# zhouxuguang/GNXRayTracer

Measured on AMD Instinct MI355X. Metric: Mrays/sec + wall-clock to 1024spp, dragon Cornell 1920×1080, higher is better.
Workload: dtype f32; 1 GPU; cfg3: Cornell + synthetic 100000-tri mesh (stand-in for absent dragon.3d), Glass+Metal, PathIntegrator maxDepth 8 rr 1 spatial, Halton(1024), 1920x1080; passes_in_flight=4, sub_passes=56, spp_rendered=1024, gather=n/a, world_size=1, backend=none, devices_visible=1

## Files before the change

### gnxraytracer_amd/csrc/api_render.hip.h

```cpp
#pragma once

struct TraceLaunch {
    int entries;
    int lds_entries;
    bool spill_needed;
    size_t lds;
    int n_top;
    int blocks;
};
static TraceLaunch trace_launch(const gnxr_scene *s, bool wide, bool spheres, long long total) {
    TraceLaunch t;
    t.entries = wide ? s->cs.stack4_need + 1 : s->cs.bvh_max_depth + 2;
    const int per_cu = g_trace_blocks_per_cu;
    const size_t fixed_b = wide ? (size_t)(kRayRecDwords + (spheres ? 1 : 0)) * kRqStride * sizeof(int) + (size_t)kTopCache * 128 + 128 : 0;
    t.lds_entries = std::min(std::min(t.entries, Knobs::trace_lds_levels()), std::max(2, (int)(((160 * 1024) / per_cu - 1024 - fixed_b) / (kBlock * sizeof(int)))));
    t.spill_needed = t.entries > t.lds_entries;
    t.lds = (size_t)t.lds_entries * kBlock * sizeof(int) + fixed_b;
    t.n_top = (int)std::min<size_t>(kTopCache, s->cs.root4 >= 0 ? s->cs.nodes4.size() : 0);
    t.blocks = (int)std::min<long long>((long long)g_num_cus * per_cu, (total + kBlock - 1) / kBlock);
    return t;
}

static int count_local_rows(const gnxr_render_params *p) {
    int rows = 0;
// ... 144 lines not shown
        return GNXR_ERR_INVALID;
    }
    return GNXR_OK;
}

int RenderState::reserve(const RenderPlan &pl) {
    const size_t cap = pl.cap, nrec = pl.nrec;
    int rc;
#define AL(f) if ((rc = f.alloc(cap)) != GNXR_OK) return rc;
    for (int i = 0; i < kRecGroups; ++i) {
        const size_t per_slot = i < 2 ? 1 : (i < 4 ? nrec : (pl.direct ? nrec : 1));
        if ((rc = rec[i].alloc(cap * per_slot * kRS)) != GNXR_OK) return rc;
    }
    if ((rc = mis_Y.alloc(cap * (pl.direct ? nrec : 1))) != GNXR_OK) return rc;
    AL(L) AL(hit) AL(queue_a) AL(queue_b) AL(queue_nee) AL(queue_c0) AL(queue_c1) AL(queue_c2) AL(queue_c3) AL(pflags) AL(pclass) AL(nee_vis)
    if (pl.whitted) {
        const size_t nl = (size_t)std::max(1, pl.n_records), md = (size_t)std::max(1, pl.p.max_depth);
        if ((rc = wh_rec.alloc(cap * nl)) ||
            (rc = wh_o.alloc(cap * md)) || (rc = wh_d.alloc(cap * md)) || (rc = wh_L.alloc(cap * md)) || (rc = wh_w.alloc(cap * md)) ||
            (rc = wh_pdf.alloc(cap * md)) || (rc = vol_vs.alloc(cap)))
            return rc;
        if (pl.textured_scene && ((rc = wh_rxo.alloc(cap * (md + 1))) || (rc = wh_rxd.alloc(cap * (md + 1))) || (rc = wh_ryo.alloc(cap * (md + 1))) || (rc = wh_ryd.alloc(cap * (md + 1)))))
            return rc;
    }
    if (pl.volpath) {
        AL(vol_n1) AL(vol_f) AL(vol_Li) AL(vol_Tr) AL(vol_Ld) AL(vol_mres) AL(vol_vs) AL(vol_state)
        AL(vol_Lout) AL(vol_alt_state) AL(vol_orig) AL(vol_alt_orig) AL(vol_newslot)
        for (int i = 0; i < kVolPackF4; ++i) AL(vol_alt[i])
        for (int i = 0; i < kRecGroups; ++i) if ((rc = vol_alt_rec[i].alloc(cap * kRS)) != GNXR_OK) return rc;
    }
#undef AL
    if ((rc = trace_spill.alloc((size_t)g_num_cus * g_trace_blocks_per_cu * kBlock * (size_t)pl.spill_entries * 2)) != GNXR_OK) return rc;
    if (!pl.caller_rays && (rc = accum.alloc(pl.npix)) != GNXR_OK) return rc;
    const int max_tiles = (int)((cap + kCompactTile - 1) / kCompactTile);
    if ((rc = tile_counts.alloc((size_t)5 * max_tiles)) != GNXR_OK) return rc;
    if (pl.n_views > 0 && (rc = view_cams.alloc((size_t)pl.n_views)) != GNXR_OK) return rc;
    return GNXR_OK;
}

unsigned long long RenderState::state_bytes(const RenderPlan &pl) {
    const unsigned long long per_slot = (2ull * kRecGroups + 2) * sizeof(float4) + 8ull * sizeof(int) + 2 + sizeof(unsigned int);
    return (unsigned long long)pl.cap * per_slot + (pl.volpath ? (unsigned long long)pl.cap * (6ull * sizeof(float4) + sizeof(int4) + 1) : 0ull);
}

PathArrays RenderState::path_arrays() {
    PathArrays pa;
    float4 *rec_primary[kRecGroups];
    record_ptrs(rec, rec_primary);
    pa.bind_records(rec_primary);
    pa.mis_Y = mis_Y.p;
    pa.L = L.p; pa.hit = hit.p; pa.pflags = pflags.p; pa.pclass = pclass.p; pa.nee_vis = nee_vis.p;
    return pa;
}
VolArrays RenderState::vol_arrays() {
    VolArrays va;
    float4 *rec_primary[kRecGroups];
    record_ptrs(rec, rec_primary);
    va.bind_records(rec_primary);
    va.mis_Y = mis_Y.p;
    va.vs = vol_vs.p; va.n1 = vol_n1.p; va.f = vol_f.p;
    va.Li = vol_Li.p; va.Tr = vol_Tr.p; va.Ld = vol_Ld.p; va.mres = vol_mres.p; va.state = vol_state.p;
    va.orig = vol_orig.p; va.Lout = vol_Lout.p;
    return va;
}
WhittedArrays RenderState::whitted_arrays(const RenderPlan &pl, int n_lights) {
    WhittedArrays wa;
    wa.ws = vol_vs.p; wa.fr_o = wh_o.p; wa.fr_d = wh_d.p; wa.fr_L = wh_L.p; wa.fr_w = wh_w.p; wa.fr_pdf = wh_pdf.p;
    wa.fr_rxo = wh_rxo.p; wa.fr_rxd = wh_rxd.p; wa.fr_ryo = wh_ryo.p; wa.fr_ryd = wh_ryd.p;
    wa.cap = (int)pl.cap; wa.n_lights = n_lights; wa.n_records = pl.n_records;
    wa.start_dim = pl.wmode == WM_DIRECT_ALL ? 5 + 2 * (pl.p.max_depth * n_lights * 2) : 5;
    return wa;
}
VolPackSet RenderState::pack_set(bool alt) {
    VolPackSet ps;
    if (!alt) {
// ... 68 lines not shown
        const int dlds_entries = std::min(std::min(entries, Knobs::trace_lds_levels()), std::max(2, (int)(((160 * 1024) / dper_cu - 1024 - dfixed) / (2 * kBlock * sizeof(int)))));
        const int dspill_levels = std::max(0, entries - dlds_entries);
        const size_t dlds = (size_t)2 * dlds_entries * kBlock * sizeof(int) + dfixed;
        const int dn_top = (int)std::min<size_t>(kTopCacheD, s->cs.root4 >= 0 ? s->cs.nodes4.size() : 0);
        const int dblocks = (int)std::min<long long>((long long)g_num_cus * dper_cu, (total + 2 * kBlock - 1) / (2 * kBlock));
#define GX_TRACE4D(S, P) hipLaunchKernelGGL((k_trace4d<S, P>), dim3(std::max(1, dblocks)), dim3(kBlock), dlds, stream, sc, pa, w, &dctr->cursor, dctr, dlds_entries, dspill_levels, st.trace_spill.p, chunk, dn_top)
        if (spheres) { if (dspill_levels > 0) GX_TRACE4D(true, true); else GX_TRACE4D(true, false); }
        else { if (dspill_levels > 0) GX_TRACE4D(false, true); else GX_TRACE4D(false, false); }
#undef GX_TRACE4D
    } else
#endif
    if (wide) {
        if (spheres) { if (count_wide) GX_TRACE4_CS(true, true); else GX_TRACE4_CS(false, true); }
        else { if (count_wide) GX_TRACE4_CS(true, false); else GX_TRACE4_CS(false, false); }
    } else {
        const bool cnt = counting || count_wide;
        if (spheres) { if (cnt) GX_TRACE(true, false, true); else GX_TRACE(false, false, true); }
        else { if (cnt) GX_TRACE(true, false, false); else GX_TRACE(false, false, false); }
    }
#undef GX_TRACE4_CS
#undef GX_TRACE4
#undef GX_TRACE
    if (timing) timer.end(stream);
    if (count_rays) {
        rays_closest += (unsigned long long)w.n_closest + (unsigned long long)n_mis;
        rays_any += (unsigned long long)n_sh;
        rays_mis += (unsigned long long)n_mis;
    }
    ++launches;
}

void RenderRun::compact(int mode, const int *qin, int nin, const unsigned char *keys, int nout, int nscatter, unsigned int *totals, int *o0, int *o1, int *o2, int *o3, int split,
                        const unsigned *n_dev) {
    int tiles = (nin + kCompactTile - 1) / kCompactTile;
    int g = std::max(1, std::min(tiles, g_num_cus * g_grid_bpc));
    unsigned int *tc = st.tile_counts.p;
    const bool hitclass = mode == COMPACT_HITCLASS;
    const int *hit = hitclass ? (const int *)st.hit.p : nullptr;
    const unsigned char *cls = hitclass ? (const unsigned char *)s->tri_class.p : nullptr;
    unsigned char *keys_out = hitclass ? st.pclass.p : nullptr;
#define GX_COUNT(M, N, SPLIT) hipLaunchKernelGGL((k_compact_count<M, N>), dim3(g), dim3(kCompactBlock), 0, stream, qin, nin, keys, tc, tiles, hit, cls, keys_out, SPLIT, n_dev)
#define GX_SCATTER(M, N, O3) hipLaunchKernelGGL((k_compact_scatter<M, N>), dim3(g), dim3(kCompactBlock), 0, stream, qin, nin, keys, (const unsigned int *)tc, tiles, o0, o1, o2, O3, n_dev)
    if (mode == COMPACT_FLAGS && nout == 5) GX_COUNT(COMPACT_FLAGS, 5, split);
    else if (mode == COMPACT_FLAGS) GX_COUNT(COMPACT_FLAGS, 4, 0);
    else if (hitclass) { if (nout == 4) GX_COUNT(COMPACT_HITCLASS, 4, 0); else GX_COUNT(COMPACT_HITCLASS, 3, 0); }
    else if (nout == 4) GX_COUNT(COMPACT_CLASS, 4, 0);
    else GX_COUNT(COMPACT_CLASS, 3, 0);
    hipLaunchKernelGGL(k_compact_scan, dim3(nout), dim3(1024), 0, stream, tc, tiles, totals, n_dev);
    if (mode == COMPACT_FLAGS && nscatter == 3) GX_SCATTER(COMPACT_FLAGS, 3, (int *)nullptr);
    else if (mode == COMPACT_FLAGS) GX_SCATTER(COMPACT_FLAGS, 2, (int *)nullptr);
    else if (nscatter == 4) GX_SCATTER(COMPACT_CLASS, 4, o3);
    else GX_SCATTER(COMPACT_CLASS, 3, (int *)nullptr);
#undef GX_SCATTER
#undef GX_COUNT
    launches += 3;
}

int RenderRun::shade_stage(const int *q_in, int n, int *q_out, const unsigned *n_dev) {
    if (timing) timer.begin(2, stream);
    const int class_mask = pl.class_mask;
    const bool escape_queue = pl.escape_queue;
    const int n_classes = ((class_mask & 8) || escape_queue) ? 4 : 3;
    compact(COMPACT_HITCLASS, q_in, n, st.pclass.p, n_classes, n_classes, &dctr->q_class[0], st.queue_c0.p, st.queue_c1.p, st.queue_c2.p, st.queue_c3.p, 0, n_dev);
    int *qc[4] = {st.queue_c0.p, st.queue_c1.p, st.queue_c2.p, st.queue_c3.p};
    dim3 g(grid_for(n, Knobs::shade_blocks_per_cu())), b(kBlock);
    const int sdims = std::min<int>(Knobs::shade_lds_dims(), (int)s->cs.prime_sums.size() - 1);
    const int snperm = sdims > 0 ? s->cs.prime_sums[sdims] : 0;
    const bool shade_lds_tabs = Knobs::shade_lds_tables();
    const int lmats = (shade_lds_tabs && s->cs.materials.size() <= 12) ? (int)s->cs.materials.size() : 0;
    const int llights = (shade_lds_tabs && n_lights > 0 && n_lights <= 16) ? n_lights : 0;
    const size_t slds = (sdims > 0 ? ((((size_t)snperm * 2 + 15) & ~(size_t)15) + (size_t)sdims * 32) : 0) + (size_t)lmats * sizeof(DMaterial) + (size_t)llights * sizeof(DLight);
    const int shade_streams = Knobs::shade_streams();
    const int n_class_kernels = 1 + ((class_mask & 2) ? 1 : 0) + ((class_mask & 4) ? 1 : 0) + (((class_mask & 8) || escape_queue) ? 1 : 0);
    const bool fork = (shade_streams < 0 ? n_class_kernels >= 3 : (shade_streams != 0 && n_class_kernels >= 2)) && s->aux_stream[0] && s->aux_stream[1];
    hipStream_t cst[4] = {stream, stream, stream, stream};
    if (fork) {
        HIP_TRY(hipEventRecord(s->ev_fork, stream));
        HIP_TRY(hipStreamWaitEvent(s->aux_stream[0], s->ev_fork, 0));
        HIP_TRY(hipStreamWaitEvent(s->aux_stream[1], s->ev_fork, 0));
        cst[1] = s->aux_stream[0]; cst[2] = s->aux_stream[1]; cst[3] = s->aux_stream[1];
    }
    const bool area_only = pl.area_only, area_env_only = pl.area_env_only;
#define GX_SHADE_K(K, C) hipLaunchKernelGGL(K, g, b, slds, cst[C], sc, r, pa, (const int *)qc[C], (const unsigned int *)&dctr->q_class[C], sdims, snperm, lmats, llights)
#define GX_SHADE(LMV, LTV, C) do { if (spheres) GX_SHADE_K((k_shade<LMV, LTV, true>), C); else GX_SHADE_K((k_shade<LMV, LTV, false>), C); } while (0)
#define GX_SHADE_TEX(LTV) do { if (spheres) GX_SHADE_K((k_shade<LM_ALL, LTV, true, true>), 3); else GX_SHADE_K((k_shade<LM_ALL, LTV, false, true>), 3); } while (0)
    if (area_only) {
        GX_SHADE(LM_DIFFUSE, LT_AREA, 0);
        if (class_mask & 2) GX_SHADE(LM_GLOSSY, LT_AREA, 1);
// ... 60 lines not shown
    RenderState &st = run.st;
    const RenderPlan &pl = run.pl;
    hipStream_t stream = run.stream;
    Counters *dctr = run.dctr;
    const size_t half = pl.half;
    struct Sub { long long u0; int kk; };
    std::vector<Sub> subs;
    for (long long u0 = pl.unit_begin; u0 < pl.unit_end; u0 += pl.k) subs.push_back(Sub{u0, (int)std::min<long long>(pl.k, pl.unit_end - u0)});
    const int R = pl.in_flight;
    struct Region { int sub = -1, started = -1; long long paths = 0; } reg[kMaxRegions];
    const int lag = std::max(1, std::min(gnxr_scene::kRing - 2, Knobs::loop_lag() >= 0 ? Knobs::loop_lag() : 2));
    const int stagger = Knobs::pipe_cut() >= 0 ? Knobs::pipe_cut() : std::max(1, (pl.p.max_depth + 2 + lag + R - 1) / R);
    int *qbuf[2] = {st.queue_a.p, st.queue_b.p};
    int in_idx = 0;
    const unsigned *cnt_ptr = &dctr->n_queue;
    size_t next_sub = 0, done_subs = 0;
    int iter = 0, last_start = -(1 << 20), newest_seen = -1;
    int ring_iter[gnxr_scene::kRing];
    for (int &v : ring_iter) v = -1;
    Counters seen;
    memset(&seen, 0, sizeof(seen));
    long long guard = 0;
    while (done_subs < subs.size()) {
        {
            int oldest_needed = iter - 1 - lag;
            for (int j = newest_seen + 1; j <= oldest_needed; ++j) {
                const int slot = j % gnxr_scene::kRing;
                if (j >= 0 && ring_iter[slot] == j) HIP_TRY(hipEventSynchronize(s->ring_ev[slot]));
            }
            for (int j = iter - 1; j > newest_seen; --j) {
                const int slot = ((j % gnxr_scene::kRing) + gnxr_scene::kRing) % gnxr_scene::kRing;
                if (j < 0 || ring_iter[slot] != j) continue;
                const hipError_t q = hipEventQuery(s->ring_ev[slot]);
                if (q == hipSuccess) { seen = s->h_ring[slot]; newest_seen = j; break; }
                if (q != hipErrorNotReady) { set_error("HIP runtime error in the path loop: hipEventQuery: %s", hipGetErrorString(q)); return hip_status(q); }
                (void)hipGetLastError();
            }
        }
        for (bool progress = true; progress;) {
            progress = false;
            for (int rg = 0; rg < R; ++rg) {
                Region &g = reg[rg];
                if (g.sub >= 0 && (run.src || g.sub == (int)done_subs) && newest_seen > g.started && seen.region_alive[rg] == 0) {
                    run.resolve(run.pa.at((size_t)rg * half), subs[g.sub].u0, subs[g.sub].kk);
                    ++run.launches; ++run.passes; ++done_subs;
                    g.sub = -1;
                    progress = true;
                }
            }
        }
        if (done_subs == subs.size()) break;
        bool any_active = false;
        long long n_upper = 0;
        for (int rg = 0; rg < R; ++rg) {
            const Region &g = reg[rg];
            if (g.sub < 0) continue;
            any_active = true;
            n_upper += newest_seen > g.started ? std::min<long long>(g.paths, seen.region_alive[rg]) : g.paths;
        }
        const int out_idx = 1 - in_idx;
        if (any_active) {
            if (int rc = run.shade_stage(qbuf[in_idx], (int)n_upper, qbuf[out_idx], cnt_ptr)) return rc;
            hipLaunchKernelGGL(k_loop_tail, dim3(1), dim3(64), 0, stream, (const int *)qbuf[out_idx], dctr, R, (int)half, (unsigned)iter);
            ++run.launches;
            const int slot = iter % gnxr_scene::kRing;
            HIP_TRY(hipMemcpyAsync(&s->h_ring[slot], dctr, sizeof(Counters), hipMemcpyDeviceToHost, stream));
            HIP_TRY(hipEventRecord(s->ring_ev[slot], stream));
// ... 51 lines not shown
    hipLaunchKernelGGL(k_whitted_init, dim3(grid_for(n_paths)), dim3(kBlock), 0, stream, pa, wa, n_paths);
    ++run.launches;
    if (textured) {
        if (run.views) hipLaunchKernelGGL(k_whitted_init_diff_views, dim3(grid_for(n_paths)), dim3(kBlock), 0, stream, sc, r, (const DCamera *)st.view_cams.p, pa, wa, n_paths);
        else hipLaunchKernelGGL(k_whitted_init_diff, dim3(grid_for(n_paths)), dim3(kBlock), 0, stream, sc, r, pa, wa, n_paths);
        ++run.launches;
    }
    int n = n_paths, n_cl = n_paths, n_shp = 0, guard = 0;
    const int *q_in = nullptr, *q_cl = nullptr;
    int *q_cur = st.queue_a.p, *q_other = st.queue_b.p;
    unsigned long long *d_shadow = &dctr->whitted_shadow;
    while (n > 0) {
        if (n_shp > 0) {
            hipLaunchKernelGGL(k_whitted_expand, dim3(grid_for((long long)n_shp * n_records)), dim3(kBlock), 0, stream, (const int *)st.queue_nee.p, n_shp, n_records, (int)pl.cap, st.wh_rec.p);
            ++run.launches;
        }
        run.launch_trace(TraceWork{q_cl, n_cl, st.wh_rec.p, n_shp * n_records}, 0, 0);
        if (run.timing) run.timer.begin(2, stream);
#define GX_WH2(MODEV, LTV, SPHV)                                                                                                                     \
    do {                                                                                                                                             \
        if (textured) hipLaunchKernelGGL((k_whitted_step<MODEV, LTV, SPHV, true>), dim3(grid_for(n)), dim3(kBlock), 0, stream, sc, r, pa, wa, q_in, n, d_shadow); \
        else hipLaunchKernelGGL((k_whitted_step<MODEV, LTV, SPHV>), dim3(grid_for(n)), dim3(kBlock), 0, stream, sc, r, pa, wa, q_in, n, d_shadow);   \
    } while (0)
#define GX_WH(LTV, SPHV) do { if (pl.wmode == WM_WHITTED) GX_WH2(WM_WHITTED, LTV, SPHV); else if (pl.wmode == WM_DIRECT_ONE) GX_WH2(WM_DIRECT_ONE, LTV, SPHV); else GX_WH2(WM_DIRECT_ALL, LTV, SPHV); } while (0)
        if (pl.area_only) { if (run.spheres) GX_WH(LT_AREA, true); else GX_WH(LT_AREA, false); }
        else { if (run.spheres) GX_WH(LT_ALL, true); else GX_WH(LT_ALL, false); }
#undef GX_WH
#undef GX_WH2
        ++run.launches;
        run.compact(COMPACT_FLAGS, q_in, n, st.pflags.p, 4, 3, &dctr->q_next, q_cur, st.queue_nee.p, st.queue_c0.p);
        if (run.timing) run.timer.end(stream);
        HIP_TRY(hipMemcpyAsync(run.s->h_counters, dctr, sizeof(Counters), hipMemcpyDeviceToHost, stream));
        HIP_TRY(hipStreamSynchronize(stream));
        n = (int)run.s->h_counters->q_next;
        n_shp = (int)run.s->h_counters->q_nee;
        n_cl = (int)run.s->h_counters->q_shadow;
        q_cl = st.queue_c0.p;
        q_in = q_cur;
        std::swap(q_cur, q_other);
        if (++guard > (1 << 20)) { set_error("path loop did not terminate"); return GNXR_ERR_INVALID; }
    }
    return GNXR_OK;
}

static int run_volpath_pass(RenderRun &run, long long u0, int kk) {
    gnxr_scene *s = run.s;
    RenderState &st = run.st;
    const RenderPlan &pl = run.pl;
    hipStream_t stream = run.stream;
    Counters *dctr = run.dctr;
    const DScene &sc = run.sc;
    const DRender &r = run.r;
    const DMediaTables &mt = run.mt;
    const PathArrays &pa = run.pa;
    const VolArrays &va = run.va;
    const int n_paths = (int)(pl.unit * kk), class_mask = pl.class_mask, nL = run.n_lights;
    int n = n_paths, guard = 0;
    const int *q_in = nullptr;
    int *q_cur = st.queue_a.p, *q_other = st.queue_b.p;
    hipLaunchKernelGGL(k_vol_init, dim3(grid_for(n_paths)), dim3(kBlock), 0, stream, pa, va, n_paths);
    ++run.launches;
    int n_media = r.cam.medium >= 0 ? n : 0;
    const int *q_media = nullptr;
    if (run.list_media) {
        run.compact(COMPACT_FLAGS, nullptr, n, st.pflags.p, 4, 2, &dctr->q_next, q_cur, st.queue_nee.p, nullptr);
        HIP_TRY(hipMemcpyAsync(s->h_counters, dctr, sizeof(Counters), hipMemcpyDeviceToHost, stream));
        HIP_TRY(hipStreamSynchronize(stream));
        n_media = (int)s->h_counters->q_nee;
        q_media = st.queue_nee.p;
    }
    bool in_alt = false;
    long long span = n_paths;
    run.bind_set(st.pack_set(false));
    while (n > 0) {
        run.launch_trace(TraceWork{q_in, n, nullptr, 0}, 0, 0);
        if (n_media > 0) {
            (void)hipMemsetAsync(&dctr->cursor, 0, sizeof(unsigned int), stream);
            int blocks = (int)std::min<long long>((long long)g_num_cus * 8, ((long long)n_media + kBlock - 1) / kBlock);
            const int vm_cap = Knobs::volmedia_step_cap();
            if (run.timing) run.timer.begin(1, stream);
            const long long mwaves = (long long)blocks * (kBlock / 64);
            const int mchunk = (int)std::min<long long>(kMediaChunk, std::max<long long>(64, ((n_media + mwaves - 1) / mwaves + 63) / 64 * 64));
            if (run.count_wide) hipLaunchKernelGGL(k_vol_media<true>, dim3(blocks), dim3(kBlock), (size_t)kVmRecDwords * kVmStride * sizeof(int), stream, sc, mt, pa, va, q_media, n_media, &dctr->cursor, mchunk, dctr, vm_cap);
            else hipLaunchKernelGGL(k_vol_media<false>, dim3(blocks), dim3(kBlock), (size_t)kVmRecDwords * kVmStride * sizeof(int), stream, sc, mt, pa, va, q_media, n_media, &dctr->cursor, mchunk, dctr, vm_cap);
            run.media_segments += (unsigned long long)n_media;
            if (run.timing) run.timer.end(stream);
            ++run.launches;
        }
        if (run.timing) run.timer.begin(2, stream);
        run.compact(COMPACT_CLASS, q_in, n, va.state, 3, 3, &dctr->q_class[0], st.queue_c0.p, st.queue_c1.p, st.queue_c2.p);
        {
            int *qc[3] = {st.queue_c0.p, st.queue_c1.p, st.queue_c2.p};
            const int vmats = s->cs.materials.size() <= 12 ? (int)s->cs.materials.size() : 0, vlights = (nL > 0 && nL <= 16) ? nL : 0;
            const size_t vlds = (size_t)vmats * sizeof(DMaterial) + (size_t)vlights * sizeof(DLight);
#define GX_VS_K(K, ST) hipLaunchKernelGGL(K, dim3(grid_for(n, 32)), dim3(kBlock), vlds, stream, sc, mt, r, pa, va, (const int *)qc[ST], (const unsigned int *)&dctr->q_class[ST], vmats, vlights)
#define GX_VS(LMV, LTV) do { GX_VS_K((k_vol_step<LMV, LTV, VS_MAIN>), VS_MAIN); GX_VS_K((k_vol_step<LMV, LTV, VS_SHADOW>), VS_SHADOW); GX_VS_K((k_vol_step<LMV, LTV, VS_MIS>), VS_MIS); } while (0)
#define GX_VST(LTV) do { GX_VS_K((k_vol_step<LM_ALL, LTV, VS_MAIN, true>), VS_MAIN); GX_VS_K((k_vol_step<LM_ALL, LTV, VS_SHADOW, true>), VS_SHADOW); GX_VS_K((k_vol_step<LM_ALL, LTV, VS_MIS, true>), VS_MIS); } while (0)
            if (pl.textured_scene) { if (pl.area_only) GX_VST(LT_AREA); else GX_VST(LT_ALL); }
            else if (pl.area_only) { if (class_mask <= 1) GX_VS(LM_DIFFUSE, LT_AREA); else if (class_mask <= 3) GX_VS(LM_GLOSSY, LT_AREA); else GX_VS(LM_ALL, LT_AREA); }
            else { if (class_mask <= 1) GX_VS(LM_DIFFUSE, LT_ALL); else if (class_mask <= 3) GX_VS(LM_GLOSSY, LT_ALL); else GX_VS(LM_ALL, LT_ALL); }
#undef GX_VST
#undef GX_VS
#undef GX_VS_K
            run.launches += 2;
        }
        ++run.launches;
        run.compact(COMPACT_FLAGS, q_in, n, st.pflags.p, 4, 2, &dctr->q_next, q_cur, st.queue_nee.p, nullptr);
        if (run.timing) run.timer.end(stream);
        HIP_TRY(hipMemcpyAsync(s->h_counters, dctr, sizeof(Counters), hipMemcpyDeviceToHost, stream));
        HIP_TRY(hipStreamSynchronize(stream));
        n = (int)s->h_counters->q_next;
        n_media = (int)s->h_counters->q_nee;
        q_media = st.queue_nee.p;
        q_in = q_cur;
        std::swap(q_cur, q_other);
        if (Knobs::vol_pack() && n >= (1 << 16) && 2ll * n <= span) {
            const VolPackSet from = st.pack_set(in_alt), to = st.pack_set(!in_alt);
            hipLaunchKernelGGL(k_vol_pack, dim3(grid_for(n)), dim3(kBlock), 0, stream, q_in, n, from, to, st.vol_newslot.p);
            if (n_media > 0) hipLaunchKernelGGL(k_vol_remap, dim3(grid_for(n_media)), dim3(kBlock), 0, stream, st.queue_nee.p, n_media, (const int *)st.vol_newslot.p);
            run.launches += 2;
            in_alt = !in_alt;
            run.bind_set(to);
            q_in = nullptr;
            span = n;
        }
        if (++guard > (1 << 20)) { set_error("path loop did not terminate"); return GNXR_ERR_INVALID; }
    }
    if (in_alt) run.bind_set(st.pack_set(false));
    return GNXR_OK;
}

static int run_passes(RenderRun &run) {
    const RenderPlan &pl = run.pl;
    for (long long u0 = pl.unit_begin; u0 < pl.unit_end; u0 += pl.k) {
        const int kk = (int)std::min<long long>(pl.k, pl.unit_end - u0);
        run.raygen(run.pa, u0, kk, run.list_media ? run.st.pflags.p : nullptr);
        ++run.launches;
        if (int rc = pl.whitted ? run_whitted_pass(run, u0, kk) : run_volpath_pass(run, u0, kk)) return rc;
        PathArrays pr = run.pa;
        if (pl.volpath) pr.L = run.st.vol_Lout.p;
        run.resolve(pr, u0, kk);
        ++run.launches;
        ++run.passes;
// ... 55 lines not shown
    sc.st.h.base32_max = (int32_t)std::min<unsigned long long>(0x7fffffffull, 0xffffffffull / ((unsigned long long)sc.st.h.stride * ((unsigned long long)p.spp * pl.max_light_samples + 1)));
    if (pl.whitted) sc.materials = s->materials_single.p + 1;
    sc.escape_class = pl.escape_queue ? 3 : 0;
    DRender r;
    memset(&r, 0, sizeof(r));
    bool views_mixed_media = false;
    if (views) {
        s->h_view_cams.resize(std::max<size_t>(s->h_view_cams.size(), (size_t)views->n_views));
        for (int v = 0; v < views->n_views; ++v) {
            s->h_view_cams[v] = make_camera(views->cameras[v], p.width, p.height, views->media ? views->media[v] : -1);
            if (s->h_view_cams[v].medium != s->h_view_cams[0].medium) views_mixed_media = true;
        }
        r.cam = s->h_view_cams[0];
    } else {
        r.cam = make_camera(s->cs.camera, p.width, p.height, s->cs.camera_medium);
    }
    r.W = p.width; r.H = p.height; r.spp = p.spp; r.max_depth = p.max_depth; r.rr_threshold = p.rr_threshold;
    r.shard_index = p.shard_index; r.shard_count = p.shard_count; r.shard_rows = p.shard_rows;
    r.npix = pl.npix;
    if (r.npix == 0) { if (stats) memset(stats, 0, sizeof(*stats)); return GNXR_OK; }
    {
        size_t free_b = 0, total_b = 0;
        const bool have_mem = hipMemGetInfo(&free_b, &total_b) == hipSuccess;
        if ((rc = pl.size_passes(s->st.L.n, have_mem, free_b)) != GNXR_OK) return rc;
    }
    if ((rc = s->st.reserve(pl)) != GNXR_OK) return rc;
    if (reserve_only) { if (stats) memset(stats, 0, sizeof(*stats)); return GNXR_OK; }

    RenderRun run(s, stream, pl, src, views, sc, r);
    run.list_media = pl.volpath && (src || views_mixed_media);
    if (views) HIP_TRY(hipMemcpyAsync(s->st.view_cams.p, s->h_view_cams.data(), (size_t)views->n_views * sizeof(DCamera), hipMemcpyHostToDevice, stream));
    if (!src) HIP_TRY(hipMemsetAsync(s->st.accum.p, 0, sizeof(float4) * r.npix, stream));
    HIP_TRY(hipMemsetAsync(run.dctr, 0, sizeof(Counters), stream));
    struct EventPair {
        hipEvent_t a = nullptr, b = nullptr;
        ~EventPair() { if (a) (void)hipEventDestroy(a); if (b) (void)hipEventDestroy(b); }
    } ev;
    HIP_TRY(hipEventCreate(&ev.a));
    HIP_TRY(hipEventCreate(&ev.b));
    HIP_TRY(hipEventRecord(ev.a, stream));
    if ((rc = pl.path_int() ? run_path_loop(run) : run_passes(run)) != GNXR_OK) return rc;
    if (!src) {
        hipLaunchKernelGGL(k_finish, dim3(grid_for(r.npix)), dim3(kBlock), 0, stream, r, (const float4 *)s->st.accum.p, (float4 *)d_rgba_out);
        ++run.launches;
    }
    HIP_TRY(hipEventRecord(ev.b, stream));
    HIP_TRY(hipMemcpyAsync(s->h_counters, run.dctr, sizeof(Counters), hipMemcpyDeviceToHost, stream));
    HIP_TRY(hipStreamSynchronize(stream));
    HIP_TRY(hipGetLastError());
    if (run.timing) run.timer.collect();
    float ms = 0;
    HIP_TRY(hipEventElapsedTime(&ms, ev.a, ev.b));
    if (stats) fill_stats(run, ms * 1e-3, std::chrono::duration<double>(std::chrono::steady_clock::now() - t_start).count(), stats);
    if (src && s->h_counters->li_bad) {
        set_error("gnxr_li_device: sample record %llu is out of range (px in [0, %d), py in [0, %d), s in [0, %d), medium in [-1, %d)); its L is (0, 0, 0, 0)",
                  ~s->h_counters->li_bad, p.width, p.height, p.spp, run.n_scene_media);
        return GNXR_ERR_INVALID;
    }
    return GNXR_OK;
}

static int render_sharded(gnxr_scene *s, const gnxr_render_params *pin, void *d_rgba_out, void *hip_stream, gnxr_stats *stats, bool reserve_only = false) {
    if (!s || !pin || !d_rgba_out) { set_error("null argument"); return GNXR_ERR_INVALID; }
    const int nd = 1 + (int)s->replicas.size();
    if (nd == 1) return render_one(s, pin, d_rgba_out, hip_stream, stats, reserve_only);
    gnxr_render_params base = *pin;
    if (base.shard_count <= 0) base.shard_count = 1;
    if (base.shard_rows <= 0) base.shard_rows = 1;
    if (base.shard_rows != 1) { set_error("multi-device rendering deals single rows: shard_rows must be 1"); return GNXR_ERR_UNSUPPORTED; }
    if (base.width <= 0 || base.height <= 0 || base.shard_index < 0 || base.shard_index >= base.shard_count) { set_error("invalid render parameters"); return GNXR_ERR_INVALID; }
    std::lock_guard<std::recursive_mutex> lock(s->render_mutex);
    const size_t npx = (size_t)base.width * base.height;
    std::vector<int> rcs(nd, GNXR_OK);
    std::vector<std::string> errs(nd);
    std::vector<gnxr_stats> sts(nd);
    std::vector<int> staged(nd, 0);
    hipStream_t caller = (hipStream_t)hip_stream;
    int rc = s->bind();
    if (rc) return rc;
    HIP_TRY(hipStreamSynchronize(caller));
    auto worker = [&](int i) {
        gnxr_scene *r = i == 0 ? s : s->replicas[i - 1].get();
        gnxr_render_params p = base;
// ... 62 lines not shown
```

### gnxraytracer_amd/csrc/api_scene.hip.h

```cpp
#pragma once

struct RenderPlan;
struct RenderState {
    DevBuf<float4> rec[kRecGroups], mis_Y;
    static void record_ptrs(DevBuf<float4> *b, float4 *g[kRecGroups]) { for (int i = 0; i < kRecGroups; ++i) g[i] = b[i].p; }
    DevBuf<float4> L, accum;
    DevBuf<int> hit, queue_a, queue_b, queue_nee, queue_c0, queue_c1, queue_c2, queue_c3;
    DevBuf<unsigned char> pflags, pclass;
    DevBuf<unsigned int> nee_vis;
    DevBuf<unsigned int> tile_counts;
    DevBuf<int> trace_spill;
    DevBuf<float4> vol_n1, vol_f, vol_Li, vol_Tr, vol_Ld, vol_mres;
    DevBuf<int4> vol_vs;
    DevBuf<unsigned char> vol_state;
    DevBuf<float4> vol_alt[kVolPackF4], vol_alt_rec[kRecGroups], vol_Lout;
    DevBuf<unsigned char> vol_alt_state;
    DevBuf<int> vol_orig, vol_alt_orig, vol_newslot;
    DevBuf<float4> wh_o, wh_d, wh_L, wh_w;
    DevBuf<float4> wh_rxo, wh_rxd, wh_ryo, wh_ryd;
    DevBuf<float> wh_pdf;
    DevBuf<int> wh_rec;
    DevBuf<DCamera> view_cams;

    int reserve(const RenderPlan &pl);
    static unsigned long long state_bytes(const RenderPlan &pl);
    PathArrays path_arrays();
    VolArrays vol_arrays();
    WhittedArrays whitted_arrays(const RenderPlan &pl, int n_lights);
    VolPackSet pack_set(bool alt);
};

struct gnxr_scene {
    CompiledScene cs;
    DevBuf<DNode> nodes;
    DevBuf<DNode4> nodes4;
    DevBuf<DTri> tris;
    DevBuf<float> leaf_boxes;
    DevBuf<uint8_t> tri_class;
    DevBuf<DSphere> spheres;
    DevBuf<DMaterial> materials, materials_single;
    DevBuf<DTexture> textures;
    DevBuf<float> tex_texels, ewa_lut, tri_uv, tri_n, tri_s;
    DevBuf<DLight> lights;
// ... 141 lines not shown
```

### gnxraytracer_amd/csrc/compact_kernel.hip.h

```cpp
#pragma once
#include "device_math.h"

namespace gnxr {

constexpr int kCompactBlock = 256;
enum CompactMode { COMPACT_FLAGS = 0, COMPACT_CLASS = 1, COMPACT_HITCLASS = 2 };

template <int MODE>
GX_DEV unsigned compact_key(const unsigned char *keys, int path) { return keys[path]; }
template <int MODE>
GX_DEV bool compact_pred(unsigned key, int o) { return MODE == COMPACT_FLAGS ? ((key >> o) & 1u) != 0 : key == (unsigned)o; }

constexpr int kCompactChunks = 8;
constexpr int kCompactTile = kCompactBlock * kCompactChunks;

template <int MODE, int NOUT>
__global__ void __launch_bounds__(kCompactBlock) k_compact_count(const int *__restrict__ q_in, int n, const unsigned char *__restrict__ keys, unsigned int *tile_counts,
                                                                 int nTiles, const int *__restrict__ hit = nullptr, const unsigned char *__restrict__ tri_class = nullptr,
                                                                 unsigned char *keys_out = nullptr, int split = 0, const unsigned *n_dev = nullptr) {
    __shared__ unsigned int wsum[NOUT][kCompactBlock / 64];
    const int lane = threadIdx.x & 63, wave = threadIdx.x >> 6;
    if (n_dev) n = (int)*n_dev;
    const int tilesUsed = n_dev ? (n + kCompactTile - 1) / kCompactTile : nTiles;
    for (int tile = blockIdx.x; tile < tilesUsed; tile += gridDim.x) {
        unsigned acc[NOUT];
#pragma unroll
        for (int o = 0; o < NOUT; ++o) acc[o] = 0;
        for (int c = 0; c < kCompactChunks; ++c) {
            const long long i = (long long)tile * kCompactTile + c * kCompactBlock + threadIdx.x;
            unsigned key = 0xffu;
            const bool valid = i < n;
            int path = -1;
            if (valid) {
                path = q_in ? q_in[i] : (int)i;
                if (MODE == COMPACT_HITCLASS) {
                    const int h = hit[path];
                    if (h >= 0) { key = tri_class[h]; keys_out[path] = (unsigned char)key; }
                    else key = keys_out[path];
                } else key = compact_key<MODE>(keys, path);
            }
#pragma unroll
            for (int o = 0; o < NOUT; ++o) {
                const bool pr = (MODE == COMPACT_FLAGS && o == 4) ? ((key & 1u) != 0 && path < split) : compact_pred<MODE>(key, o);
                acc[o] += (unsigned)__popcll(__ballot(valid && pr));
            }
        }
#pragma unroll
        for (int o = 0; o < NOUT; ++o) if (lane == 0) wsum[o][wave] = acc[o];
        __syncthreads();
        if (threadIdx.x < NOUT) {
            unsigned s = 0;
            for (int w = 0; w < kCompactBlock / 64; ++w) s += wsum[threadIdx.x][w];
            tile_counts[(size_t)threadIdx.x * nTiles + tile] = s;
        }
        __syncthreads();
    }
}

static __global__ void __launch_bounds__(1024) k_compact_scan(unsigned int *tile_counts, int nTiles, unsigned int *totals, const unsigned *n_dev = nullptr) {
    __shared__ unsigned int wtot[16];
    __shared__ unsigned int carry_s;
    unsigned int *c = tile_counts + (size_t)blockIdx.x * nTiles;
    const int lane = threadIdx.x & 63, wave = threadIdx.x >> 6;
    if (threadIdx.x == 0) carry_s = 0;
    if (n_dev) nTiles = ((int)*n_dev + kCompactTile - 1) / kCompactTile;
    __syncthreads();
    for (int base = 0; base < nTiles; base += 1024) {
        int i = base + threadIdx.x;
        unsigned v = i < nTiles ? c[i] : 0u;
        unsigned x = v;
#pragma unroll
        for (int off = 1; off < 64; off <<= 1) { unsigned y = __shfl_up(x, off); if (lane >= off) x += y; }
        if (lane == 63) wtot[wave] = x;
        __syncthreads();
        unsigned woff = 0;
        for (int w = 0; w < wave; ++w) woff += wtot[w];
        unsigned carry = carry_s;
        if (i < nTiles) c[i] = carry + woff + x - v;
        __syncthreads();
        if (threadIdx.x == 1023) carry_s = carry + woff + x;
        __syncthreads();
    }
    if (threadIdx.x == 0) totals[blockIdx.x] = carry_s;
}

template <int MODE, int NSCATTER>
__global__ void __launch_bounds__(kCompactBlock) k_compact_scatter(const int *__restrict__ q_in, int n, const unsigned char *__restrict__ keys,
                                                                   const unsigned int *__restrict__ tile_offsets, int nTiles, int *out0, int *out1, int *out2, int *out3 = nullptr,
                                                                   const unsigned *n_dev = nullptr) {
    __shared__ unsigned int wsum[NSCATTER][kCompactBlock / 64];
    const int lane = threadIdx.x & 63, wave = threadIdx.x >> 6;
    int *outs[4] = {out0, out1, out2, out3};
    if (n_dev) n = (int)*n_dev;
    const int tilesUsed = n_dev ? (n + kCompactTile - 1) / kCompactTile : nTiles;
    for (int tile = blockIdx.x; tile < tilesUsed; tile += gridDim.x) {
        unsigned base[NSCATTER];
#pragma unroll
        for (int o = 0; o < NSCATTER; ++o) base[o] = tile_offsets[(size_t)o * nTiles + tile];
        for (int c = 0; c < kCompactChunks; ++c) {
            const long long i = (long long)tile * kCompactTile + c * kCompactBlock + threadIdx.x;
            unsigned key = 0xffu;
            const bool valid = i < n;
            int path = -1;
            if (valid) { path = q_in ? q_in[i] : (int)i; key = compact_key<MODE>(keys, path); }
            unsigned long long masks[NSCATTER];
#pragma unroll
            for (int o = 0; o < NSCATTER; ++o) {
                masks[o] = __ballot(valid && compact_pred<MODE>(key, o));
                if (lane == 0) wsum[o][wave] = (unsigned)__popcll(masks[o]);
            }
            __syncthreads();
#pragma unroll
            for (int o = 0; o < NSCATTER; ++o) {
                unsigned woff = 0, tot = 0;
                for (int w = 0; w < kCompactBlock / 64; ++w) { const unsigned v = wsum[o][w]; if (w < wave) woff += v; tot += v; }
                if (valid && compact_pred<MODE>(key, o)) outs[o][base[o] + woff + (unsigned)__popcll(masks[o] & ((1ull << lane) - 1ull))] = path;
                base[o] += tot;
            }
            __syncthreads();
        }
    }
}

}
```

### gnxraytracer_amd/csrc/kernels.hip.h

```cpp
#pragma once
#include "device_bsdf.h"
#include "device_lights.h"
#include "device_texture.h"

namespace gnxr {

constexpr int kBlock = 256;

constexpr int kRS = 2;
constexpr int kRSm = 2 * kRS;
constexpr int kRecGroups = 5;
struct PathArrays {
    float4 *ray_o;
    float4 *ray_d;
    float4 *beta;
    uint2 *meta;
    float4 *L;
    int *hit;
    unsigned char *pflags;
    unsigned char *pclass;
    float4 *sh_o;
    float4 *sh_d;
    float4 *sh_X;
    float4 *nbeta;
// ... 6 lines not shown
        sh_o = g[2]; sh_d = g[2] + 1; sh_X = g[3]; nbeta = g[3] + 1;
        mis_o = g[4]; mis_d = g[4] + 1;
    }
    __device__ void store_meta(size_t i, uint32_t x, uint32_t y) const { *reinterpret_cast<uint4 *>(&meta[i * kRSm]) = make_uint4(x, y, 0u, 0u); }
    __host__ __device__ PathArrays at(size_t base) const {
        PathArrays q = *this;
        q.ray_o += base * kRS; q.ray_d += base * kRS; q.beta += base * kRS; q.meta += base * kRSm;
        q.sh_o += base * kRS; q.sh_d += base * kRS; q.sh_X += base * kRS; q.nbeta += base * kRS;
        q.mis_o += base * kRS; q.mis_d += base * kRS;
        q.mis_Y += base; q.L += base; q.hit += base; q.pflags += base; q.pclass += base; q.nee_vis += base;
        return q;
    }
};

constexpr int kMaxRegions = 8;
struct Counters {
    unsigned long long nodes, tris;
    unsigned int q_next, q_nee, q_shadow, q_mis;
    unsigned int q_low;
    unsigned int q_class[4];
    unsigned int cursor;
    unsigned long long whitted_shadow;
    unsigned long long whitted_mis;
    unsigned long long media_steps;
    unsigned long long media_cont;
    unsigned long long retests;
    unsigned long long nodes_global;
    unsigned int n_queue;
    unsigned int iter;
    unsigned int region_lb[kMaxRegions + 1];
    unsigned int region_alive[kMaxRegions];
    unsigned long long rays_continue, rays_shadow, rays_mis;
    unsigned long long li_bad;
};

struct DScene {
    const float4 *nodes;
    const float4 *nodes4;
    int root4;
    const DTri *tris;
    const unsigned char *tri_class;
    const float4 *leaf_box;
    int leaf1_from_verts;
    const DSphere *spheres;
    int n_spheres;
    int escape_class;
    const DMaterial *materials;
    DLightTables lt;
    DSamplerTables st;
};

struct DRender {
    DCamera cam;
    int W, H, spp, max_depth;
    float rr_threshold;
    int shard_index, shard_count, shard_rows;
    int npix;
};

}
#include "compact_kernel.hip.h"
#include "trace_kernel.hip.h"
namespace gnxr {

GX_DEV void local_pixel(const DRender &r, int lp, int *x, int *y) {
    int row = lp / r.W;
// ... 748 lines not shown
```

Measured before the change: 4808 Mrays/s.

## Replace three-pass queue compaction with single-pass decoupled look-back kernel

Queue compaction now runs as one kernel instead of count, scan and scatter launches. Tiles are claimed through an atomic ticket and publish aggregate and inclusive-prefix descriptors so later tiles can find their offsets by decoupled look-back. Keys are read once and predicate bits are kept in registers for the scatter. Tiles and blocks are larger, and a poll cap with a stall flag reported to the host guards against deadlock. The intent is to cut launch overhead and the second pass over queue and key memory, at the cost of spin-waiting and more complex synchronisation.

```diff
diff --git a/gnxraytracer_amd/csrc/api_render.hip.h b/gnxraytracer_amd/csrc/api_render.hip.h
--- a/gnxraytracer_amd/csrc/api_render.hip.h
+++ b/gnxraytracer_amd/csrc/api_render.hip.h
@@ -200,15 +200,23 @@
 #undef AL
     if ((rc = trace_spill.alloc((size_t)g_num_cus * g_trace_blocks_per_cu * kBlock * (size_t)pl.spill_entries * 2)) != GNXR_OK) return rc;
     if (!pl.caller_rays && (rc = accum.alloc(pl.npix)) != GNXR_OK) return rc;
-    const int max_tiles = (int)((cap + kCompactTile - 1) / kCompactTile);
-    if ((rc = tile_counts.alloc((size_t)5 * max_tiles)) != GNXR_OK) return rc;
+    const size_t max_tiles = (cap + kCompactTile - 1) / kCompactTile;
+    if (tile_desc.n < kCompactMaxOut * max_tiles || !tile_desc.p) {
+        if ((rc = tile_desc.alloc(kCompactMaxOut * max_tiles)) != GNXR_OK) return rc;
+        HIP_TRY(hipMemset(tile_desc.p, 0, tile_desc.n * sizeof(unsigned long long)));
+        HIP_TRY(hipDeviceSynchronize());
+        compact_seq = 0;
+    }
+    if ((rc = compact_ticket.alloc(2)) != GNXR_OK) return rc;
     if (pl.n_views > 0 && (rc = view_cams.alloc((size_t)pl.n_views)) != GNXR_OK) return rc;
     return GNXR_OK;
 }
 
 unsigned long long RenderState::state_bytes(const RenderPlan &pl) {
     const unsigned long long per_slot = (2ull * kRecGroups + 2) * sizeof(float4) + 8ull * sizeof(int) + 2 + sizeof(unsigned int);
-    return (unsigned long long)pl.cap * per_slot + (pl.volpath ? (unsigned long long)pl.cap * (6ull * sizeof(float4) + sizeof(int4) + 1) : 0ull);
+    const unsigned long long tiles = ((unsigned long long)pl.cap + kCompactTile - 1) / kCompactTile;
+    return (unsigned long long)pl.cap * per_slot + tiles * kCompactMaxOut * sizeof(unsigned long long) +
+           (pl.volpath ? (unsigned long long)pl.cap * (6ull * sizeof(float4) + sizeof(int4) + 1) : 0ull);
 }
 
 PathArrays RenderState::path_arrays() {
@@ -343,28 +351,31 @@
 
 void RenderRun::compact(int mode, const int *qin, int nin, const unsigned char *keys, int nout, int nscatter, unsigned int *totals, int *o0, int *o1, int *o2, int *o3, int split,
                         const unsigned *n_dev) {
-    int tiles = (nin + kCompactTile - 1) / kCompactTile;
-    int g = std::max(1, std::min(tiles, g_num_cus * g_grid_bpc));
-    unsigned int *tc = st.tile_counts.p;
+    const int tiles = (nin + kCompactTile - 1) / kCompactTile;
+    const int g = std::max(1, std::min(tiles, g_num_cus * kCompactBlocksPerCu));
+    if (st.compact_seq >= (1u << 30) - 1u) {
+        (void)hipMemsetAsync(st.tile_desc.p, 0, st.tile_desc.n * sizeof(unsigned long long), stream);
+        st.compact_seq = 0;
+    }
+    const unsigned seq = ++st.compact_seq;
+    const CompactScratch cs{st.tile_desc.p, tiles, st.compact_ticket.p + (seq & 1u), st.compact_ticket.p + ((seq + 1u) & 1u), seq};
     const bool hitclass = mode == COMPACT_HITCLASS;
     const int *hit = hitclass ? (const int *)st.hit.p : nullptr;
     const unsigned char *cls = hitclass ? (const unsigned char *)s->tri_class.p : nullptr;
-    unsigned char *keys_out = hitclass ? st.pclass.p : nullptr;
-#define GX_COUNT(M, N, SPLIT) hipLaunchKernelGGL((k_compact_count<M, N>), dim3(g), dim3(kCompactBlock), 0, stream, qin, nin, keys, tc, tiles, hit, cls, keys_out, SPLIT, n_dev)
-#define GX_SCATTER(M, N, O3) hipLaunchKernelGGL((k_compact_scatter<M, N>), dim3(g), dim3(kCompactBlock), 0, stream, qin, nin, keys, (const unsigned int *)tc, tiles, o0, o1, o2, O3, n_dev)
-    if (mode == COMPACT_FLAGS && nout == 5) GX_COUNT(COMPACT_FLAGS, 5, split);
-    else if (mode == COMPACT_FLAGS) GX_COUNT(COMPACT_FLAGS, 4, 0);
-    else if (hitclass) { if (nout == 4) GX_COUNT(COMPACT_HITCLASS, 4, 0); else GX_COUNT(COMPACT_HITCLASS, 3, 0); }
-    else if (nout == 4) GX_COUNT(COMPACT_CLASS, 4, 0);
-    else GX_COUNT(COMPACT_CLASS, 3, 0);
-    hipLaunchKernelGGL(k_compact_scan, dim3(nout), dim3(1024), 0, stream, tc, tiles, totals, n_dev);
-    if (mode == COMPACT_FLAGS && nscatter == 3) GX_SCATTER(COMPACT_FLAGS, 3, (int *)nullptr);
-    else if (mode == COMPACT_FLAGS) GX_SCATTER(COMPACT_FLAGS, 2, (int *)nullptr);
-    else if (nscatter == 4) GX_SCATTER(COMPACT_CLASS, 4, o3);
-    else GX_SCATTER(COMPACT_CLASS, 3, (int *)nullptr);
-#undef GX_SCATTER
-#undef GX_COUNT
-    launches += 3;
+#define GX_COMPACT(M, N, NS) hipLaunchKernelGGL((k_compact<M, N, NS>), dim3(g), dim3(kCompactBlock), 0, stream, qin, nin, keys, cs, totals, o0, o1, o2, o3, hit, cls, split, n_dev, dctr)
+    if (mode == COMPACT_FLAGS) {
+        if (nout == 5) { if (nscatter == 3) GX_COMPACT(COMPACT_FLAGS, 5, 3); else GX_COMPACT(COMPACT_FLAGS, 5, 2); }
+        else { if (nscatter == 3) GX_COMPACT(COMPACT_FLAGS, 4, 3); else GX_COMPACT(COMPACT_FLAGS, 4, 2); }
+    } else if (hitclass) { if (nout == 4) GX_COMPACT(COMPACT_HITCLASS, 4, 4); else GX_COMPACT(COMPACT_HITCLASS, 3, 3); }
+    else if (nout == 4) GX_COMPACT(COMPACT_CLASS, 4, 4);
+    else GX_COMPACT(COMPACT_CLASS, 3, 3);
+#undef GX_COMPACT
+    launches += 1;
+}
+static int compact_stalled(const Counters &c) {
+    if (!c.compact_stall) return GNXR_OK;
+    set_error("queue compaction: a tile waited for its predecessors beyond the poll limit (k_compact); the render was abandoned");
+    return GNXR_ERR_RUNTIME;
 }
 
 int RenderRun::shade_stage(const int *q_in, int n, int *q_out, const unsigned *n_dev) {
@@ -491,7 +502,7 @@
                 const int slot = ((j % gnxr_scene::kRing) + gnxr_scene::kRing) % gnxr_scene::kRing;
                 if (j < 0 || ring_iter[slot] != j) continue;
                 const hipError_t q = hipEventQuery(s->ring_ev[slot]);
-                if (q == hipSuccess) { seen = s->h_ring[slot]; newest_seen = j; break; }
+                if (q == hipSuccess) { seen = s->h_ring[slot]; newest_seen = j; if (int rc = compact_stalled(seen)) return rc; break; }
                 if (q != hipErrorNotReady) { set_error("HIP runtime error in the path loop: hipEventQuery: %s", hipGetErrorString(q)); return hip_status(q); }
                 (void)hipGetLastError();
             }
@@ -609,6 +620,7 @@
         if (run.timing) run.timer.end(stream);
         HIP_TRY(hipMemcpyAsync(run.s->h_counters, dctr, sizeof(Counters), hipMemcpyDeviceToHost, stream));
         HIP_TRY(hipStreamSynchronize(stream));
+        if (int rc = compact_stalled(*run.s->h_counters)) return rc;
         n = (int)run.s->h_counters->q_next;
         n_shp = (int)run.s->h_counters->q_nee;
         n_cl = (int)run.s->h_counters->q_shadow;
@@ -643,6 +655,7 @@
         run.compact(COMPACT_FLAGS, nullptr, n, st.pflags.p, 4, 2, &dctr->q_next, q_cur, st.queue_nee.p, nullptr);
         HIP_TRY(hipMemcpyAsync(s->h_counters, dctr, sizeof(Counters), hipMemcpyDeviceToHost, stream));
         HIP_TRY(hipStreamSynchronize(stream));
+        if (int rc = compact_stalled(*s->h_counters)) return rc;
         n_media = (int)s->h_counters->q_nee;
         q_media = st.queue_nee.p;
     }
@@ -686,6 +699,7 @@
         if (run.timing) run.timer.end(stream);
         HIP_TRY(hipMemcpyAsync(s->h_counters, dctr, sizeof(Counters), hipMemcpyDeviceToHost, stream));
         HIP_TRY(hipStreamSynchronize(stream));
+        if (int rc = compact_stalled(*s->h_counters)) return rc;
         n = (int)s->h_counters->q_next;
         n_media = (int)s->h_counters->q_nee;
         q_media = st.queue_nee.p;
@@ -807,6 +821,7 @@
     if (views) HIP_TRY(hipMemcpyAsync(s->st.view_cams.p, s->h_view_cams.data(), (size_t)views->n_views * sizeof(DCamera), hipMemcpyHostToDevice, stream));
     if (!src) HIP_TRY(hipMemsetAsync(s->st.accum.p, 0, sizeof(float4) * r.npix, stream));
     HIP_TRY(hipMemsetAsync(run.dctr, 0, sizeof(Counters), stream));
+    HIP_TRY(hipMemsetAsync(s->st.compact_ticket.p, 0, 2 * sizeof(unsigned int), stream));
     struct EventPair {
         hipEvent_t a = nullptr, b = nullptr;
         ~EventPair() { if (a) (void)hipEventDestroy(a); if (b) (void)hipEventDestroy(b); }
@@ -824,6 +839,7 @@
     HIP_TRY(hipStreamSynchronize(stream));
     HIP_TRY(hipGetLastError());
     if (run.timing) run.timer.collect();
+    if ((rc = compact_stalled(*s->h_counters)) != GNXR_OK) return rc;
     float ms = 0;
     HIP_TRY(hipEventElapsedTime(&ms, ev.a, ev.b));
     if (stats) fill_stats(run, ms * 1e-3, std::chrono::duration<double>(std::chrono::steady_clock::now() - t_start).count(), stats);
diff --git a/gnxraytracer_amd/csrc/api_scene.hip.h b/gnxraytracer_amd/csrc/api_scene.hip.h
--- a/gnxraytracer_amd/csrc/api_scene.hip.h
+++ b/gnxraytracer_amd/csrc/api_scene.hip.h
@@ -8,7 +8,9 @@
     DevBuf<int> hit, queue_a, queue_b, queue_nee, queue_c0, queue_c1, queue_c2, queue_c3;
     DevBuf<unsigned char> pflags, pclass;
     DevBuf<unsigned int> nee_vis;
-    DevBuf<unsigned int> tile_counts;
+    DevBuf<unsigned long long> tile_desc;
+    DevBuf<unsigned int> compact_ticket;
+    unsigned int compact_seq = 0;
     DevBuf<int> trace_spill;
     DevBuf<float4> vol_n1, vol_f, vol_Li, vol_Tr, vol_Ld, vol_mres;
     DevBuf<int4> vol_vs;
diff --git a/gnxraytracer_amd/csrc/compact_kernel.hip.h b/gnxraytracer_amd/csrc/compact_kernel.hip.h
--- a/gnxraytracer_amd/csrc/compact_kernel.hip.h
+++ b/gnxraytracer_amd/csrc/compact_kernel.hip.h
@@ -3,121 +3,159 @@
 
 namespace gnxr {
 
-constexpr int kCompactBlock = 256;
+constexpr int kCompactBlock = 512;
 enum CompactMode { COMPACT_FLAGS = 0, COMPACT_CLASS = 1, COMPACT_HITCLASS = 2 };
 
 template <int MODE>
-GX_DEV unsigned compact_key(const unsigned char *keys, int path) { return keys[path]; }
-template <int MODE>
 GX_DEV bool compact_pred(unsigned key, int o) { return MODE == COMPACT_FLAGS ? ((key >> o) & 1u) != 0 : key == (unsigned)o; }
 
-constexpr int kCompactChunks = 8;
+constexpr int kCompactChunks = 32;
 constexpr int kCompactTile = kCompactBlock * kCompactChunks;
+constexpr int kCompactWaves = kCompactBlock / 64;
+constexpr int kCompactSpan = 64 * kCompactChunks;
+constexpr int kCompactBlocksPerCu = 2;
+constexpr int kCompactGather = 8;
+constexpr unsigned kCompactPollCap = 1u << 21;
+constexpr int kCompactMaxOut = 5;
+static_assert(kCompactChunks <= 32 && kCompactChunks % kCompactGather == 0, "predicate masks are 32-bit");
+static_assert(kCompactMaxOut <= kCompactWaves, "one wave per predicate looks back");
 
-template <int MODE, int NOUT>
-__global__ void __launch_bounds__(kCompactBlock) k_compact_count(const int *__restrict__ q_in, int n, const unsigned char *__restrict__ keys, unsigned int *tile_counts,
-                                                                 int nTiles, const int *__restrict__ hit = nullptr, const unsigned char *__restrict__ tri_class = nullptr,
-                                                                 unsigned char *keys_out = nullptr, int split = 0, const unsigned *n_dev = nullptr) {
-    __shared__ unsigned int wsum[NOUT][kCompactBlock / 64];
-    const int lane = threadIdx.x & 63, wave = threadIdx.x >> 6;
-    if (n_dev) n = (int)*n_dev;
-    const int tilesUsed = n_dev ? (n + kCompactTile - 1) / kCompactTile : nTiles;
-    for (int tile = blockIdx.x; tile < tilesUsed; tile += gridDim.x) {
+enum : unsigned { COMPACT_DESC_COUNT = 1u, COMPACT_DESC_PREFIX = 2u };
+GX_DEV unsigned long long compact_desc(unsigned tag, unsigned value) { return ((unsigned long long)tag << 32) | value; }
+
+struct CompactScratch {
+    unsigned long long *desc;
+    int stride;
+    unsigned *ticket;
+    unsigned *ticket_next;
+    unsigned seq;
+};
+
+template <int MODE, int NOUT, int NSCATTER>
+__global__ void __launch_bounds__(kCompactBlock) k_compact(const int *__restrict__ q_in, int n, const unsigned char *__restrict__ keys, CompactScratch cs,
+                                                           unsigned int *totals, int *out0, int *out1, int *out2, int *out3, const int *__restrict__ hit,
+                                                           const unsigned char *__restrict__ tri_class, int split, const unsigned *n_dev, Counters *ctr) {
+    __shared__ unsigned int wtot[NOUT][kCompactWaves];
+    __shared__ unsigned int s_excl[NOUT];
+    __shared__ unsigned int s_ticket;
+    __shared__ int s_stop;
+    const int tid = threadIdx.x, lane = tid & 63, wave = tid >> 6;
+    int *outs[4] = {out0, out1, out2, out3};
+    if (n_dev) n = (int)min(*n_dev, (unsigned)n);
+    const int tilesUsed = (n + kCompactTile - 1) / kCompactTile;
+    if (blockIdx.x == 0 && tid == 0) *cs.ticket_next = 0u;
+    if (tilesUsed == 0) {
+        if (blockIdx.x == 0 && tid < NOUT) totals[tid] = 0u;
+        return;
+    }
+    if (tid == 0) s_stop = 0;
+    const unsigned tag_count = (cs.seq << 2) | COMPACT_DESC_COUNT, tag_prefix = (cs.seq << 2) | COMPACT_DESC_PREFIX;
+    for (;;) {
+        __syncthreads();
+        if (tid == 0) s_ticket = atomicAdd(cs.ticket, 1u);
+        __syncthreads();
+        const unsigned tile = s_ticket;
+        if (tile >= (unsigned)tilesUsed) break;
+        const long long base = (long long)tile * kCompactTile + wave * kCompactSpan + lane;
+        const int *q = q_in ? q_in + base : nullptr;
+        const int left = (int)min((long long)n - base, (long long)kCompactSpan);
+        int path[kCompactChunks];
+#pragma unroll
+        for (int c = 0; c < kCompactChunks; ++c) path[c] = c * 64 < left ? (q ? q[c * 64] : (int)base + c * 64) : -1;
+        unsigned m[NSCATTER];
+#pragma unroll
+        for (int o = 0; o < NSCATTER; ++o) m[o] = 0u;
         unsigned acc[NOUT];
 #pragma unroll
-        for (int o = 0; o < NOUT; ++o) acc[o] = 0;
-        for (int c = 0; c < kCompactChunks; ++c) {
-            const long long i = (long long)tile * kCompactTile + c * kCompactBlock + threadIdx.x;
-            unsigned key = 0xffu;
-            const bool valid = i < n;
-            int path = -1;
-            if (valid) {
-                path = q_in ? q_in[i] : (int)i;
-                if (MODE == COMPACT_HITCLASS) {
-                    const int h = hit[path];
-                    if (h >= 0) { key = tri_class[h]; keys_out[path] = (unsigned char)key; }
-                    else key = keys_out[path];
-                } else key = compact_key<MODE>(keys, path);
+        for (int o = 0; o < NOUT; ++o) acc[o] = 0u;
+#pragma unroll
+        for (int c0 = 0; c0 < kCompactChunks; c0 += kCompactGather) {
+            unsigned key[kCompactGather];
+            if (MODE == COMPACT_HITCLASS) {
+                int h[kCompactGather];
+#pragma unroll
+                for (int j = 0; j < kCompactGather; ++j) h[j] = path[c0 + j] >= 0 ? hit[path[c0 + j]] : -1;
+#pragma unroll
+                for (int j = 0; j < kCompactGather; ++j) key[j] = path[c0 + j] < 0 ? 0xffu : (h[j] >= 0 ? (unsigned)tri_class[h[j]] : (unsigned)keys[path[c0 + j]]);
+            } else {
+#pragma unroll
+                for (int j = 0; j < kCompactGather; ++j) key[j] = path[c0 + j] >= 0 ? (unsigned)keys[path[c0 + j]] : 0xffu;
             }
 #pragma unroll
-            for (int o = 0; o < NOUT; ++o) {
-                const bool pr = (MODE == COMPACT_FLAGS && o == 4) ? ((key & 1u) != 0 && path < split) : compact_pred<MODE>(key, o);
-                acc[o] += (unsigned)__popcll(__ballot(valid && pr));
+            for (int j = 0; j < kCompactGather; ++j) {
+                const int c = c0 + j;
+                const bool valid = path[c] >= 0;
+#pragma unroll
+                for (int o = 0; o < NOUT; ++o) {
+                    const bool pr = valid && ((MODE == COMPACT_FLAGS && o == 4) ? ((key[j] & 1u) != 0 && path[c] < split) : compact_pred<MODE>(key[j], o));
+                    if (o < NSCATTER) m[o < NSCATTER ? o : 0] |= (pr ? 1u : 0u) << c;
+                    acc[o] += (unsigned)__popcll(__ballot(pr));
+                }
             }
         }
 #pragma unroll
-        for (int o = 0; o < NOUT; ++o) if (lane == 0) wsum[o][wave] = acc[o];
+        for (int o = 0; o < NSCATTER; ++o) m[o] = (unsigned)__shfl((int)m[o], lane);
+#pragma unroll
+        for (int o = 0; o < NOUT; ++o) if (lane == 0) wtot[o][wave] = acc[o];
         __syncthreads();
-        if (threadIdx.x < NOUT) {
-            unsigned s = 0;
-            for (int w = 0; w < kCompactBlock / 64; ++w) s += wsum[threadIdx.x][w];
-            tile_counts[(size_t)threadIdx.x * nTiles + tile] = s;
+        if (wave < NOUT) {
+            const int o = wave;
+            unsigned agg = 0;
+            for (int w = 0; w < kCompactWaves; ++w) agg += wtot[o][w];
+            unsigned long long *d = cs.desc + (size_t)o * cs.stride;
+            if (lane == 0) __hip_atomic_store(&d[tile], compact_desc(tile == 0 ? tag_prefix : tag_count, agg), __ATOMIC_RELAXED, __HIP_MEMORY_SCOPE_AGENT);
+            unsigned excl = 0, polls = 0;
+            bool stalled = false;
+            long long j = (long long)tile - 1;
+            while (j >= 0) {
+                const long long idx = j - lane;
+                const unsigned long long w = idx >= 0 ? __hip_atomic_load(&d[idx], __ATOMIC_RELAXED, __HIP_MEMORY_SCOPE_AGENT) : compact_desc(tag_prefix, 0u);
+                const unsigned tag = (unsigned)(w >> 32);
+                const unsigned long long has_prefix = __ballot(tag == tag_prefix), not_ready = __ballot(tag != tag_prefix && tag != tag_count);
+                const int first = has_prefix ? __ffsll((long long)has_prefix) - 1 : 63;
+                const unsigned long long needed = first >= 63 ? ~0ull : ((2ull << first) - 1ull);
+                if (not_ready & needed) {
+                    if (++polls > kCompactPollCap) { stalled = true; break; }
+                    __builtin_amdgcn_s_sleep(2);
+                    continue;
+                }
+                unsigned sum = lane <= first ? (unsigned)w : 0u;
+#pragma unroll
+                for (int off = 32; off > 0; off >>= 1) sum += __shfl_xor(sum, off);
+                excl += sum;
+                if (has_prefix) break;
+                j -= 64;
+            }
+            if (lane == 0) {
+                if (stalled) {
+                    s_stop = 1;
+                    atomicOr(&ctr->compact_stall, 1u);
+                    __hip_atomic_store(cs.ticket, 0x80000000u, __ATOMIC_RELAXED, __HIP_MEMORY_SCOPE_AGENT);
+                } else {
+                    s_excl[o] = excl;
+                    if (tile > 0) __hip_atomic_store(&d[tile], compact_desc(tag_prefix, excl + agg), __ATOMIC_RELAXED, __HIP_MEMORY_SCOPE_AGENT);
+                    if (tile == (unsigned)tilesUsed - 1u) totals[o] = excl + agg;
+                }
+            }
         }
         __syncthreads();
-    }
-}
-
-static __global__ void __launch_bounds__(1024) k_compact_scan(unsigned int *tile_counts, int nTiles, unsigned int *totals, const unsigned *n_dev = nullptr) {
-    __shared__ unsigned int wtot[16];
-    __shared__ unsigned int carry_s;
-    unsigned int *c = tile_counts + (size_t)blockIdx.x * nTiles;
-    const int lane = threadIdx.x & 63, wave = threadIdx.x >> 6;
-    if (threadIdx.x == 0) carry_s = 0;
-    if (n_dev) nTiles = ((int)*n_dev + kCompactTile - 1) / kCompactTile;
-    __syncthreads();
-    for (int base = 0; base < nTiles; base += 1024) {
-        int i = base + threadIdx.x;
-        unsigned v = i < nTiles ? c[i] : 0u;
-        unsigned x = v;
+        if (s_stop) return;
+        unsigned run[NSCATTER];
 #pragma unroll
-        for (int off = 1; off < 64; off <<= 1) { unsigned y = __shfl_up(x, off); if (lane >= off) x += y; }
-        if (lane == 63) wtot[wave] = x;
-        __syncthreads();
-        unsigned woff = 0;
-        for (int w = 0; w < wave; ++w) woff += wtot[w];
-        unsigned carry = carry_s;
-        if (i < nTiles) c[i] = carry + woff + x - v;
-        __syncthreads();
-        if (threadIdx.x == 1023) carry_s = carry + woff + x;
-        __syncthreads();
-    }
-    if (threadIdx.x == 0) totals[blockIdx.x] = carry_s;
-}
-
-template <int MODE, int NSCATTER>
-__global__ void __launch_bounds__(kCompactBlock) k_compact_scatter(const int *__restrict__ q_in, int n, const unsigned char *__restrict__ keys,
-                                                                   const unsigned int *__restrict__ tile_offsets, int nTiles, int *out0, int *out1, int *out2, int *out3 = nullptr,
-                                                                   const unsigned *n_dev = nullptr) {
-    __shared__ unsigned int wsum[NSCATTER][kCompactBlock / 64];
-    const int lane = threadIdx.x & 63, wave = threadIdx.x >> 6;
-    int *outs[4] = {out0, out1, out2, out3};
-    if (n_dev) n = (int)*n_dev;
-    const int tilesUsed = n_dev ? (n + kCompactTile - 1) / kCompactTile : nTiles;
-    for (int tile = blockIdx.x; tile < tilesUsed; tile += gridDim.x) {
-        unsigned base[NSCATTER];
+        for (int o = 0; o < NSCATTER; ++o) {
+            run[o] = s_excl[o];
+            for (int w = 0; w < wave; ++w) run[o] += wtot[o][w];
+        }
 #pragma unroll
-        for (int o = 0; o < NSCATTER; ++o) base[o] = tile_offsets[(size_t)o * nTiles + tile];
         for (int c = 0; c < kCompactChunks; ++c) {
-            const long long i = (long long)tile * kCompactTile + c * kCompactBlock + threadIdx.x;
-            unsigned key = 0xffu;
-            const bool valid = i < n;
-            int path = -1;
-            if (valid) { path = q_in ? q_in[i] : (int)i; key = compact_key<MODE>(keys, path); }
-            unsigned long long masks[NSCATTER];
 #pragma unroll
             for (int o = 0; o < NSCATTER; ++o) {
-                masks[o] = __ballot(valid && compact_pred<MODE>(key, o));
-                if (lane == 0) wsum[o][wave] = (unsigned)__popcll(masks[o]);
+                const bool pr = ((m[o] >> c) & 1u) != 0;
+                const unsigned long long b = __ballot(pr);
+                const unsigned rank = __builtin_amdgcn_mbcnt_hi((unsigned)(b >> 32), __builtin_amdgcn_mbcnt_lo((unsigned)b, 0u));
+                if (pr) outs[o][run[o] + rank] = path[c];
+                run[o] += (unsigned)__popcll(b);
             }
-            __syncthreads();
-#pragma unroll
-            for (int o = 0; o < NSCATTER; ++o) {
-                unsigned woff = 0, tot = 0;
-                for (int w = 0; w < kCompactBlock / 64; ++w) { const unsigned v = wsum[o][w]; if (w < wave) woff += v; tot += v; }
-                if (valid && compact_pred<MODE>(key, o)) outs[o][base[o] + woff + (unsigned)__popcll(masks[o] & ((1ull << lane) - 1ull))] = path;
-                base[o] += tot;
-            }
-            __syncthreads();
         }
     }
 }
diff --git a/gnxraytracer_amd/csrc/kernels.hip.h b/gnxraytracer_amd/csrc/kernels.hip.h
--- a/gnxraytracer_amd/csrc/kernels.hip.h
+++ b/gnxraytracer_amd/csrc/kernels.hip.h
@@ -62,6 +62,7 @@
     unsigned int region_alive[kMaxRegions];
     unsigned long long rays_continue, rays_shadow, rays_mis;
     unsigned long long li_bad;
+    unsigned int compact_stall;
 };
 
 struct DScene {
```

New measurement: 4890 Mrays/s, median of 6. 1.7% higher.
